# GameTechDev/Intel-Texture-Works-Plugin

Measured on AMD Instinct MI355X. Metric: Mpixels/s encode (BC1/BC3/BC7/BC6H) at 4k x 4k; bit-exact vs the oracle under the pinned ISPC sse/avx-target arithmetic model (no ispc binary exists here; sensitivity of that model: profiles/arith_sensitivity.txt), higher is better.
Workload: dtype f32; 1 GPU; bc7_slow: BC7 GetProfile_slow on ONE synthetic 4096x4096 RGBA8 surface, weak-sharded over 1 GPU(s) by block-row bands (4096 texel rows per rank), texels resident in HBM, device-pointer C ABI call; blocks_per_gpu=1048576, ranks_seen_by_rccl=1, device=gfx950:sramecc+:xnack- / AMD Radeon Graphics / 256 CUs / 2400 MHz, lib=itw-amd 0.1 gfx950 arith=x86-lut-nr contract=off

## Files before the change

intel-texture-works-plugin_amd/csrc/bc7.hip:

```cpp
#include <atomic>
#include <cstdlib>
#include <cstring>
#include <type_traits>
#include "bc7_exact.hpp"
#include "kernels.hpp"
#include "host_rt.hpp"
#ifdef ITW_TEST_HOOKS
#include "../../include/itw_test_hooks.h"
#endif

namespace itw {

#define BCN_TABLE_QUAL __device__ const
#include "bc7_f02_schedule.h"
#undef BCN_TABLE_QUAL

constexpr int LANE_PAL_LEVELS = 24;
constexpr int TPB = 256;
constexpr float INV255 = 1.0f / 255.0f;
constexpr int32_t ERR_MAX = 0x7fffffff;
enum Family { F_MODES02 = 0, F_MODES13 = 1, F_MODE7 = 2, F_MODES456 = 3 };

struct ModeTraits { int pairs, bits, ch; };
__device__ __forceinline__ constexpr ModeTraits traits(int mode)
// ... 1190 lines not shown
    const int32_t chunk = sel_chunk(sel, chunk_i);
    const int32_t nact = (!FAM7 && rgb_list) ? *rgb_count : nblocks;
    if (chunk * TPB >= nact) return;
    Lane ln;
    ln.T = stage_seed_tables_fast(s_seed16, s_seed32, threadIdx.x, TPB);
    __syncthreads();
    const int32_t gid = chunk * TPB + threadIdx.x;
    const bool live = gid < nact;
    const int32_t slot = live ? gid : nact - 1;
    const int32_t b = (!FAM7 && rgb_list) ? rgb_list[slot] : slot;
    ln.keys = nullptr;
    ln.pal = s_pal + threadIdx.x;
    load_block<VEC16>(ln.tx, src, stride, blocks_x, b);
    const int kind = tasks.kind[t];
    Win wa, wb;
    if (!FAM7 && kind == WK_SCAN02) {
        search_02(ln, S, wa, wb);
        if (live) { wins4[(int64_t)wide_win_slot(0) * nblocks + b] = pack_win(wa); if (!S.skip_mode2) wins4[(int64_t)wide_win_slot(2) * nblocks + b] = pack_win(wb); }
    } else if (!FAM7) {
        if (RANKED_LISTS && ranked13) search_two_subset<false, 3, 2>(ln, S, wa, wb); else search_two_subset<false, 3, 0>(ln, S, wa, wb);
        if (live) { wins4[(int64_t)wide_win_slot(1) * nblocks + b] = pack_win(wa); wins4[(int64_t)wide_win_slot(3) * nblocks + b] = pack_win(wb); }
    } else {
        if (S.channels == 4) { if (RANKED_LISTS && ranked7) search_two_subset<true, 4, 2>(ln, S, wa, wb); else search_two_subset<true, 4, 0>(ln, S, wa, wb); }
        else                 { if (RANKED_LISTS && ranked7) search_two_subset<true, 3, 2>(ln, S, wa, wb); else search_two_subset<true, 3, 0>(ln, S, wa, wb); }
        if (live) wins4[(int64_t)wide_win_slot(7) * nblocks + b] = pack_win(wa);
    }
}

__device__ __forceinline__ int32_t append_to_list(int32_t* __restrict__ list, int32_t* __restrict__ count, bool need, int32_t b)
{
    const unsigned long long m = __ballot(need);
    int32_t pos = -1;
    if (m) {
        const int lane = (int)(threadIdx.x & 63u);
        int32_t base = 0;
        if (lane == 0) base = atomicAdd(count, (int32_t)__popcll(m));
        base = __shfl(base, 0);
        if (need) { pos = base + (int32_t)__popcll(m & ((1ull << lane) - 1ull)); list[pos] = b; }
    }
    return pos;
}
__device__ __forceinline__ void append_to_rotation_lists(int32_t (*s_cnt)[4], const RotRegion& R, bool need0, bool need1, bool need2, int32_t b)
{
    const int lane = (int)__builtin_amdgcn_mbcnt_hi(~0u, __builtin_amdgcn_mbcnt_lo(~0u, 0u));
    const int wave = __builtin_amdgcn_readfirstlane((int)(threadIdx.x >> 6));
    const unsigned long long m0 = __ballot(need0), m1 = __ballot(need1), m2 = __ballot(need2);
    if (lane < 3) s_cnt[wave][lane] = (int32_t)__popcll(lane == 0 ? m0 : (lane == 1 ? m1 : m2));
    __syncthreads();
    if (threadIdx.x < 3u) {
        int32_t t = 0;
#pragma unroll
        for (int w = 0; w < TPB / 64; w++) t += s_cnt[w][lane];
        int32_t base = t ? atomicAdd(R.counts + lane, t) : 0;
#pragma unroll
        for (int w = 0; w < TPB / 64; w++) { const int32_t c = s_cnt[w][lane]; s_cnt[w][lane] = base; base += c; }
    }
    __syncthreads();
    const unsigned long long below = (1ull << lane) - 1ull;
    if (need0) R.lists[                      s_cnt[wave][0] + (int32_t)__popcll(m0 & below)] = b;
    if (need1) R.lists[(int64_t)R.cap     + s_cnt[wave][1] + (int32_t)__popcll(m1 & below)] = b;
    if (need2) R.lists[(int64_t)R.cap * 2 + s_cnt[wave][2] + (int32_t)__popcll(m2 & below)] = b;
}

__device__ __forceinline__ bool mode6_cannot_win(Lane& ln)
{
    if (__all(ln.best_err == 0)) return true;
    IStats<3> full;
    stats_int<3>(full, ln.tx.pl, whole_block());
    const float d = __builtin_amdgcn_sqrtf(subset_residual_bound(full) * rcp_of_count(16)) * 0.999999f - BOUND_SLACK3[16];
    const float e = fmaxf(d, 0.0f);
    const float lb = e * e * 0.999999f;
    return __all(lb >= (float)ln.best_err);
}

#ifndef FINISH_ALL_WAVES
#define FINISH_ALL_WAVES 2
#endif
#ifndef BOUND_BAIL_AFTER
#define BOUND_BAIL_AFTER 4
#endif
#ifndef BOUND_BAIL_LANES
#define BOUND_BAIL_LANES 40
#endif
template <bool VEC16, int PHASE>
__global__ void __launch_bounds__(TPB) __attribute__((amdgpu_waves_per_eu(FINISH_ALL_WAVES, FINISH_ALL_WAVES)))
bc7_finish_all(const uint8_t* __restrict__ src, int64_t stride, int32_t blocks_x, int32_t nblocks, uint8_t* __restrict__ dst,
               const uint32_t* __restrict__ wins4, const bc7_enc_settings S, int32_t* __restrict__ inc_err,
               const int32_t* __restrict__ in_list, const int32_t* __restrict__ in_count, int32_t* __restrict__ out_list, int32_t* __restrict__ out_count,
               int32_t* __restrict__ out_list7, int32_t* __restrict__ out_count7, const ChunkSel sel,
               const uint4* __restrict__ in_compact, uint4* __restrict__ out_compact, const RotRegion R)
{
    constexpr bool LISTED = PHASE == 2 || PHASE == 4 || PHASE == 5 || PHASE == 7 || PHASE == 8;
    constexpr bool DO02 = PHASE == 0 || PHASE == 2 || PHASE == 3 || PHASE == 5 || PHASE == 9;
    constexpr bool TAIL3 = PHASE == 3 || PHASE == 10;
    constexpr bool DO13 = PHASE == 0 || PHASE == 2 || PHASE == 4;
    constexpr bool DO7 = PHASE == 0 || PHASE == 1;
    constexpr bool DO456 = PHASE == 0 || PHASE == 1 || PHASE == 3 || PHASE == 6;
    __shared__ unsigned short s_seed16[2048];
    __shared__ uint32_t s_seed32[2048];
    __shared__ uint2 s_pal[LANE_PAL_LEVELS * TPB];
    __shared__ int32_t s_at[TAIL3 ? TPB / 64 : 1][64];
    __shared__ int32_t s_listed[TPB / 64];
    __shared__ int32_t s_rot[PHASE == 9 ? TPB / 64 : 1][4];
    if (sel.gate && *sel.gate != sel.want) return;
    const int32_t nact = LISTED ? *in_count : nblocks;
    const int32_t chunk = LISTED ? (int32_t)blockIdx.x : sel_chunk(sel, (int32_t)blockIdx.x);
    if (chunk * TPB >= nact) return;
    Lane ln;
    ln.T = stage_seed_tables_fast(s_seed16, s_seed32, threadIdx.x, TPB);
    __syncthreads();
    const int32_t gid = chunk * TPB + threadIdx.x;
    const bool live = gid < nact;
    const int32_t slot = live ? gid : nact - 1;
    const int32_t b = LISTED ? in_list[slot] : slot;
    ln.keys = nullptr;
    ln.pal = s_pal + threadIdx.x;
    if (LISTED && in_compact) load_block_compact(ln.tx, in_compact, slot); else load_block<VEC16>(ln.tx, src, stride, blocks_x, b);
    ln.best_err = ERR_MAX;
    ln.best[0] = ln.best[1] = ln.best[2] = ln.best[3] = 0u;
    ln.improved = false;
    ln.opaque_err = 0;
    if (S.channels == 4) {
        uint32_t e = 0;
#pragma unroll
        for (int d = 0; d < 4; d++) { const uint32_t x = ~ln.tx.pl[3][d]; e = udot4(x, x, e); }
        ln.opaque_err = (int32_t)e;
    }
    const bool on13 = S.mode_selection[1];
    int32_t e_alpha = ERR_MAX;
    if (PHASE == 2 || PHASE == 5) e_alpha = inc_err[b];
    if (PHASE == 4 || PHASE == 7 || PHASE == 8 || PHASE == 10) ln.best_err = inc_err[b];
    Win w;
    if (DO02 && S.mode_selection[0]) {
        unpack_win(w, wins4[(int64_t)wide_win_slot(0) * nblocks + b]);
        refine_and_commit<0>(ln, w, S.refineIterations[0], S.channels);
        if (!S.skip_mode2) { ln.tx.fence(); unpack_win(w, wins4[(int64_t)wide_win_slot(2) * nblocks + b]); refine_and_commit<2>(ln, w, S.refineIterations[2], S.channels); }
    }
    const int32_t e02 = ln.best_err;
    if (PHASE == 9) {
        if (live) { inc_err[b] = e02; R.words[b] = ~0ull; }
        ln.tx.fence();
        IStats<3> full;
        stats_int<3>(full, ln.tx.pl, whole_block());
        const float lim = (float)e02 - 0.5f;
        const bool on45 = live && S.mode_selection[2];
        bool need[3];
#pragma unroll
        for (int r = 0; r < 3; r++) need[r] = on45 && r >= S.mode45_channel0 && !(rotation_bound(r, full) >= lim);
        append_to_rotation_lists(s_rot, R, need[0], need[1], need[2], b);
    }
    if (PHASE == 10) {
        const unsigned long long v = R.words[b];
        const int32_t e = (int32_t)(v >> 32);
        if (v != ~0ull && e < ln.best_err) {
            const uint4 p = R.payload[(int64_t)((v >> ROT_WORD_ROT_SHIFT) & 3ull) * R.cap + (int64_t)(v & ROT_WORD_POS_MASK)];
            ln.best_err = e; ln.improved = true;
            ln.best[0] = p.x; ln.best[1] = p.y; ln.best[2] = p.z; ln.best[3] = p.w;
        }
        ln.tx.fence();
        if (S.mode_selection[3] && !mode6_cannot_win(ln)) mode_6<3>(ln, S);
    }
    if (DO13 && PHASE != 4) {
        if (on13 && S.fastSkipTreshold_mode1 > 0) { ln.tx.fence(); unpack_win(w, wins4[(int64_t)wide_win_slot(1) * nblocks + b]); refine_and_commit<1>(ln, w, S.refineIterations[1], S.channels); }
        if (on13 && S.fastSkipTreshold_mode3 > 0) { ln.tx.fence(); unpack_win(w, wins4[(int64_t)wide_win_slot(3) * nblocks + b]); refine_and_commit<3>(ln, w, S.refineIterations[3], S.channels); }
    }
    if (PHASE == 4) {
        const int parts = list_scan_parts(nact, nblocks);
        if (S.fastSkipTreshold_mode1 > 0) { ln.tx.fence(); merge_packed_parts<3, 3>(w, ln, wins4 + (int64_t)wide_win_slot(1) * nblocks, nact, parts, slot); refine_and_commit<1>(ln, w, S.refineIterations[1], S.channels); }
        if (S.fastSkipTreshold_mode3 > 0) { ln.tx.fence(); merge_packed_parts<3, 3>(w, ln, wins4 + (int64_t)wide_win_slot(3) * nblocks, nact, parts, slot); refine_and_commit<3>(ln, w, S.refineIterations[3], S.channels); }
    }
    bool redo = false;
    if (PHASE == 8) {
        const unsigned long long* pw = reinterpret_cast<const unsigned long long*>(wins4) + 2 * (int64_t)slot;
        const int32_t inc = ln.best_err;
        const bool heavy = pw[0] == PAIR_WORD_HEAVY;
        redo = !heavy && *out_count7 != 0;
        const bool use = !heavy && !redo;
        const unsigned long long v1 = (use && S.fastSkipTreshold_mode1 > 0) ? pw[0] : ~0ull, v3 = (use && S.fastSkipTreshold_mode3 > 0) ? pw[1] : ~0ull;
        if (v1 != ~0ull) {
            ln.tx.fence();
            w.err = (int32_t)(v1 >> 32); w.key = (int32_t)(uint32_t)v1; w.shape = w.key & 63;
            const bool open = w.err + ln.opaque_err >= inc;
            const int32_t before = ln.best_err;
            refine_and_commit<1>(ln, w, S.refineIterations[1], S.channels);
            redo = redo || (open && ln.best_err < before);
        }
        if (v3 != ~0ull) {
            ln.tx.fence();
            w.err = (int32_t)(v3 >> 32); w.key = (int32_t)(uint32_t)v3; w.shape = w.key & 63;
            const bool open = w.err + ln.opaque_err >= inc;
            const int32_t before = ln.best_err;
            refine_and_commit<3>(ln, w, S.refineIterations[3], S.channels);
            redo = redo || (open && ln.best_err < before);
        }
        append_to_list(out_list, out_count, live && redo, b);
    }
    if (PHASE == 7) {
        const int parts = list_scan_parts(nact, nblocks);
        ln.tx.fence();
        merge_packed_parts<4, 4>(w, ln, wins4 + (int64_t)wide_win_slot(7) * nblocks, nact, parts, slot);
        refine_and_commit<7>(ln, w, S.refineIterations[7], S.channels);
    }
    if (DO7 && on13 && S.fastSkipTreshold_mode7 > 0) { ln.tx.fence(); unpack_win(w, wins4[(int64_t)wide_win_slot(7) * nblocks + b]); refine_and_commit<7>(ln, w, S.refineIterations[7], S.channels); }
    if (DO456) {
        ln.tx.fence();
        if (S.mode_selection[2]) modes_45(ln, S);
        if (S.mode_selection[3]) {
            if (S.channels == 4) mode_6<4>(ln, S);
            else if (!mode6_cannot_win(ln)) mode_6<3>(ln, S);
        }
    }
    if (PHASE == 1) {
        if (live) inc_err[b] = ln.best_err;
        append_to_list(out_list, out_count, live && ln.opaque_err <= ln.best_err, b);
    }
    if (PHASE == 6) {
        const bool rgb = ln.opaque_err <= ln.best_err;
        if (live) inc_err[b] = rgb ? ln.best_err : ln.best_err + 1;
        append_to_list(out_list, out_count, live && rgb, b);
        append_to_list(out_list7, out_count7, live && !rgb, b);
    }
    if (TAIL3 || PHASE == 5) {
        int32_t inc;
        if (TAIL3) inc = ln.best_err + (ln.best_err < e02 ? 1 : 0);
        else            inc = (e02 <= e_alpha) ? e02 : e_alpha + 1;
        if (live) inc_err[b] = inc;
        ln.tx.fence();
        IStats<3> full;
        stats_int<3>(full, ln.tx.pl, whole_block());
        const float lim = (float)(inc - ln.opaque_err) - 0.5f;
        const float lim7 = (float)inc - 0.5f;
        const bool with7 = PHASE == 5 && out_list7 != nullptr;
        const PairTarget* target = nullptr;
        if (TAIL3) target = reinterpret_cast<const PairTarget*>(out_count + (PAIR_CTR_TARGET - PAIR_CTR_LIST));
        const bool pairs = TAIL3 && target->P.words != nullptr;
        bool need = !live, need7 = !live || !with7;
        unsigned long long mine = 0, any = 0;
#pragma unroll 1
        for (int shape = 0; shape < 64; shape++) {
            if (!pairs) {
                if (__all(need && need7)) break;
                if (shape == BOUND_BAIL_AFTER && __popcll(__ballot(need && need7)) >= BOUND_BAIL_LANES) { need = true; need7 = true; break; }
            }
            const float lb = two_subset_bound(shape, ln.tx.pl, full);
            const bool in = !(lb >= lim);
            need = need || in;
            need7 = need7 || !(lb >= lim7);
            if (pairs) {
                mine |= (live && in) ? (1ull << shape) : 0ull;
                any |= __ballot(live && in) ? (1ull << shape) : 0ull;
            }
        }
        int32_t pos = -1;
        if (!pairs) pos = append_to_list(out_list, out_count, live && need, b);
        else {
            const int lane = (int)__builtin_amdgcn_mbcnt_hi(~0u, __builtin_amdgcn_mbcnt_lo(~0u, 0u));
            const int wave = __builtin_amdgcn_readfirstlane((int)(threadIdx.x >> 6));
            const PairRegion P = target->P;
            const bool heavy = __popcll(mine) > PAIR_MAX_PER_BLOCK;
            if (heavy) mine = 0;
            const unsigned long long listed = __ballot(live && need);
            int32_t k = 0;
            for (unsigned long long rest = any; rest; rest &= rest - 1ull) {
                const int shape = __builtin_amdgcn_readfirstlane((int)__builtin_ctzll(rest));
                const int32_t c = (int32_t)__popcll(__ballot((mine >> shape) & 1ull));
                k = (lane == shape) ? c : k;
            }
            s_at[wave][lane] = k;
            if (lane == 0) s_listed[wave] = (int32_t)__popcll(listed);
            __syncthreads();
            if (threadIdx.x < 64u) {
                int32_t t = 0;
#pragma unroll
                for (int w = 0; w < TPB / 64; w++) t += s_at[w][lane];
                int32_t base = t ? atomicAdd(P.ctr + lane, t) : 0;
                if (base + t > P.cap) { P.ctr[PAIR_CTR_OVERFLOW] = 1; base = -1; }
#pragma unroll
                for (int w = 0; w < TPB / 64; w++) { const int32_t c = s_at[w][lane]; s_at[w][lane] = base; base = base < 0 ? -1 : base + c; }
            } else if (threadIdx.x == 64u) {
                int32_t t = 0;
#pragma unroll
                for (int w = 0; w < TPB / 64; w++) t += s_listed[w];
                int32_t base = t ? atomicAdd(out_count, t) : 0;
#pragma unroll
                for (int w = 0; w < TPB / 64; w++) { const int32_t c = s_listed[w]; s_listed[w] = base; base += c; }
            }
            __syncthreads();
            if (live && need) { pos = s_listed[wave] + (int32_t)__popcll(listed & ((1ull << lane) - 1ull)); out_list[pos] = b; }
            if (pos >= 0) { P.words[2 * (int64_t)pos] = heavy ? PAIR_WORD_HEAVY : ~0ull; P.words[2 * (int64_t)pos + 1] = ~0ull; }
            append_to_list(target->redo, P.ctr + PAIR_CTR_REDO, heavy, b);
            const int32_t at = s_at[wave][lane];
            for (unsigned long long rest = any; rest; rest &= rest - 1ull) {
                const int shape = __builtin_amdgcn_readfirstlane((int)__builtin_ctzll(rest));
                const bool in = (mine >> shape) & 1ull;
                const unsigned long long m = __ballot(in);
                const int32_t base = __builtin_amdgcn_readlane(at, shape);
                if (in && base >= 0) P.buckets[(int64_t)shape * P.cap + base + (int32_t)__popcll(m & ((1ull << lane) - 1ull))] = pos;
            }
        }
        if (out_compact && pos >= 0) {
            uint4* c = out_compact + (int64_t)pos * 4;
#pragma unroll
            for (int y = 0; y < 4; y++) c[y] = make_uint4(ln.tx.w[y * 4 + 0], ln.tx.w[y * 4 + 1], ln.tx.w[y * 4 + 2], ln.tx.w[y * 4 + 3]);
        }
        if (with7) append_to_list(out_list7, out_count7, live && need7, b);
    }
    bool store = live;
    if (PHASE == 2 || PHASE == 5) store = store && ln.best_err <= e_alpha;
    if (PHASE == 4 || PHASE == 7 || PHASE == 10) store = store && ln.improved;
    if (PHASE == 8) store = store && ln.improved && !redo;
    if ((PHASE == 4 || PHASE == 8) && store) inc_err[b] = ln.best_err;
    if (store) {
        uint32_t* d = reinterpret_cast<uint32_t*>(dst + (int64_t)b * 16);
        if (VEC16) *reinterpret_cast<uint4*>(d) = make_uint4(ln.best[0], ln.best[1], ln.best[2], ln.best[3]);
        else { d[0] = ln.best[0]; d[1] = ln.best[1]; d[2] = ln.best[2]; d[3] = ln.best[3]; }
    }
}

template <bool VEC16>
__global__ void __launch_bounds__(TPB)
bc7_pilot_estimate(const uint8_t* __restrict__ src, int64_t stride, int32_t blocks_x, int32_t nblocks, const uint32_t* __restrict__ wins4,
                   const int skip_mode2, const ChunkSel sel, int32_t* __restrict__ counters , const int32_t thr256,
                   int32_t* __restrict__ flag, int32_t* __restrict__ host_counts )
{
    const int32_t chunk = sel_chunk(sel, (int32_t)blockIdx.x * 8 + 3);
    if (chunk * TPB < nblocks) {
        const int32_t gid = chunk * TPB + threadIdx.x;
        const bool live = gid < nblocks;
        const int32_t b = live ? gid : nblocks - 1;
        Tex tx;
        load_block<VEC16>(tx, src, stride, blocks_x, b);
        Win w0, w2;
        unpack_win(w0, wins4[(int64_t)wide_win_slot(0) * nblocks + b]);
        unpack_win(w2, skip_mode2 ? 0xffffffffu : wins4[(int64_t)wide_win_slot(2) * nblocks + b]);
        const int32_t e = min(w0.err, w2.err);
        IStats<3> full;
        stats_int<3>(full, tx.pl, whole_block());
        const float lim = (float)e - 0.5f;
        bool need = !live;
#pragma unroll 1
        for (int shape = 0; shape < 64; shape++) {
            if (__all(need)) break;
            if (shape == BOUND_BAIL_AFTER && __popcll(__ballot(need)) >= BOUND_BAIL_LANES) { need = true; break; }
            need = need || !(two_subset_bound(shape, tx.pl, full) >= lim);
        }
        const unsigned long long ml = __ballot(live && need), mt = __ballot(live);
        if ((threadIdx.x & 63u) == 0u) { atomicAdd(counters + PILOT_LISTED, (int32_t)__popcll(ml)); atomicAdd(counters + PILOT_SAMPLED, (int32_t)__popcll(mt)); }
    }
    __syncthreads();
    if (threadIdx.x == 0) {
        __threadfence();
        if (atomicAdd(counters + PILOT_DONE, 1) == (int32_t)gridDim.x - 1) {
            __threadfence();
            const int64_t listed = atomicAdd(counters + PILOT_LISTED, 0), sampled = atomicAdd(counters + PILOT_SAMPLED, 0);
            *flag = (listed * 256 <= (int64_t)thr256 * sampled) ? 1 : 0;
            if (host_counts) { host_counts[0] = (int32_t)listed; host_counts[1] = (int32_t)sampled; __threadfence_system(); }
        }
    }
}

__global__ void __launch_bounds__(TPB) bc7_bounded_setup(int32_t* __restrict__ counters, const PairTarget t0, const PairTarget t1)
{
    for (int i = (int)threadIdx.x; i < CTR_WORDS + 2 * PAIR_CTR_WORDS; i += TPB) {
        const int j = i < CTR_WORDS ? 0 : (i - CTR_WORDS) % PAIR_CTR_WORDS;
        if (i < CTR_WORDS || j < PAIR_CTR_TARGET) counters[i] = 0;
    }
    if (threadIdx.x == 0) {
        *reinterpret_cast<PairTarget*>(counters + CTR_WORDS + PAIR_CTR_TARGET) = t0;
        *reinterpret_cast<PairTarget*>(counters + CTR_WORDS + PAIR_CTR_WORDS + PAIR_CTR_TARGET) = t1;
    }
}


__global__ void __launch_bounds__(TPB) __attribute__((amdgpu_waves_per_eu(4, 4)))
bc7_pair_scan(const uint8_t* __restrict__ src, int64_t stride, int32_t blocks_x, const int32_t* __restrict__ list, const uint4* __restrict__ compact,
              const bc7_enc_settings S, const PairRegion P)
{
    __shared__ unsigned short s_seed16[2048];
    __shared__ uint32_t s_seed32[2048];
    __shared__ uint2 s_pal[12 * TPB];
    __shared__ int32_t s_first[65];
    if (P.ctr[PAIR_CTR_OVERFLOW]) return;
    if (threadIdx.x == 0) {
        int32_t t = 0;
        for (int s = 0; s < 64; s++) { s_first[s] = t; t += (P.ctr[s] + 63) >> 6; }
        s_first[64] = t;
    }
    __syncthreads();
    const int32_t total = s_first[64];
    const int32_t wpb = TPB / 64;
    if ((int32_t)blockIdx.x * wpb >= total) return;
    Lane ln;
    ln.T = stage_seed_tables_fast(s_seed16, s_seed32, threadIdx.x, TPB);
    __syncthreads();
    ln.keys = nullptr;
    ln.pal = s_pal + threadIdx.x;
    const int lane = (int)(threadIdx.x & 63u);
    const bool on_a = S.fastSkipTreshold_mode1 > 0, on_b = S.fastSkipTreshold_mode3 > 0;
    int shape = 0;
// ... 573 lines not shown
    uint32_t* wins4;
    int32_t* alpha_err;
    int32_t* list_rgb;
    int32_t* list13;
    int32_t* list7;
    int32_t* ctr;
};
static Fused fused_context(const Bc7Launch& L, const Bc7Modes& M, float* workspace, const Bc7Aux* aux)
{
    Fused C{L, M, aux, fused_layout((size_t)L.n, fused_needs(M)), (int32_t)(((int64_t)L.n + TPB - 1) / TPB)};
    C.wins4 = reinterpret_cast<uint32_t*>(workspace);
    auto at = [&](size_t word) { return reinterpret_cast<int32_t*>(C.wins4 + word); };
    C.alpha_err = at(C.W.inc); C.list_rgb = at(C.W.list0); C.list13 = at(C.W.list1); C.list7 = at(C.W.list2); C.ctr = at(C.W.counts);
    return C;
}

struct Span { ChunkSel sel; int32_t cnt; hipStream_t s; uint32_t* wins; int32_t rows; };
struct BlockList { const int32_t* list; const int32_t* count; const uint4* compact; };
static const ChunkSel ALL_CHUNKS{0, 1, 0, nullptr, 0};
static const BlockList NO_LIST{nullptr, nullptr, nullptr};

struct Band {
    ChunkSel sel; int32_t cnt; hipStream_t s; int32_t* list; int32_t* count; uint32_t* wins; int32_t rows;
    int32_t* list_rgb; int32_t* count_rgb; int32_t* list7; int32_t* count7;
    uint4* compact; PairRegion P; int32_t* redo; RotRegion R;
};
static bool two_bands(const Fused& C) { return bc7_bands() > 1 && C.aux && !C.aux->single && C.aux->stream && C.nchunks >= 32; }
static Band make_band(const Fused& C, bool two, int k, hipStream_t s)
{
    int32_t stripe = C.nchunks / 16;
    stripe = stripe < 1 ? 1 : (stripe > 64 ? 64 : stripe);
    const int32_t stripes = (C.nchunks + stripe - 1) / stripe;
    Band B{};
    B.sel = ChunkSel{two ? 1 : 0, stripe, k, nullptr, 0};
    B.cnt = two ? ((stripes + 1 - k) / 2) * stripe : C.nchunks;
    B.s = s;
    B.wins = two ? C.wins4 + C.W.band[k].wins : C.wins4;
    B.rows = two ? B.cnt * TPB : C.L.n;
    return B;
}
static Span surface(const Fused& C) { return Span{ALL_CHUNKS, C.nchunks, C.L.st, C.wins4, C.L.n}; }
static Span band_chunks(const Fused& C, const Band& B) { return Span{B.sel, B.cnt, B.s, C.wins4, C.L.n}; }
static Span band_list(const Band& B) { return Span{ALL_CHUNKS, B.cnt, B.s, B.wins, B.rows}; }
static Span band_list_surface_rows(const Fused& C, const Band& B) { return Span{ALL_CHUNKS, B.cnt, B.s, C.wins4, C.L.n}; }

enum { SCAN02 = 1, SCAN13 = 2 };
static void scan_rgb(const Fused& C, int families, const Span& sp, const BlockList& in = NO_LIST, int32_t split = 0)
{
    const Bc7Launch& L = C.L;
    ScanTasks T{};
    if (C.M.on13 && (families & SCAN13)) T.kind[T.n++] = WK_SCAN13;
    if (C.M.on02 && (families & SCAN02)) T.kind[T.n++] = WK_SCAN02;
    if (T.n == 0) return;
    const int32_t c8 = ((sp.cnt + 7) / 8) * 8;
    const int32_t grain = c8 < 256 ? c8 : 256;
    const int32_t groups = (c8 + grain - 1) / grain;
    const dim3 grid((unsigned)(groups * grain * T.n));
    with_bools(L.vec, C.M.r13, [&](auto V, auto K) {
        hipLaunchKernelGGL((bc7_scan_all<decltype(V)::value, decltype(K)::value, false>), grid, dim3(TPB), 0, sp.s, L.src, L.stride, L.bx, sp.rows, sp.wins, L.S, T,
                           C.M.r13 ? 1 : 0, C.M.r7 ? 1 : 0, sp.cnt, grain, in.list, in.count, split, sp.sel, in.compact);
    });
}
static void scan_7(const Fused& C, const Span& sp, const BlockList& in = NO_LIST, int32_t split = 0)
{
    const Bc7Launch& L = C.L;
    if (!C.M.on7) return;
    const ScanTasks T7{1, {WK_SCAN7}};
    const int32_t chunks8 = ((sp.cnt + 7) / 8) * 8;
    with_bools(L.vec, C.M.r7, [&](auto V, auto K) {
        hipLaunchKernelGGL((bc7_scan_all<decltype(V)::value, decltype(K)::value, true>), dim3((unsigned)chunks8), dim3(TPB), 0, sp.s, L.src, L.stride, L.bx, sp.rows, sp.wins, L.S, T7,
                           C.M.r13 ? 1 : 0, C.M.r7 ? 1 : 0, sp.cnt, chunks8, in.list, in.count, split, ALL_CHUNKS, (const uint4*)nullptr);
    });
}
struct FinishIO {
    const int32_t* in_list = nullptr; const int32_t* in_count = nullptr; const uint4* in_compact = nullptr;
    int32_t* out_list = nullptr; int32_t* out_count = nullptr; uint4* out_compact = nullptr;
    int32_t* out_list7 = nullptr; int32_t* out_count7 = nullptr;
    RotRegion rot{nullptr, nullptr, nullptr, nullptr, 0};
    FinishIO& in(const int32_t* l, const int32_t* c, const uint4* texels = nullptr) { in_list = l; in_count = c; in_compact = texels; return *this; }
    FinishIO& out(int32_t* l, int32_t* c, uint4* texels = nullptr) { out_list = l; out_count = c; out_compact = texels; return *this; }
    FinishIO& out7(int32_t* l, int32_t* c) { out_list7 = l; out_count7 = c; return *this; }
    FinishIO& rotations(const RotRegion& r) { rot = r; return *this; }
};
template <int PH>
static void finish(const Fused& C, const Span& sp, const FinishIO& io = FinishIO())
{
    const Bc7Launch& L = C.L;
    const int32_t* band0 = C.ctr + CTR_WORDS + PAIR_CTR_LIST;
    if ((PH == 3 || PH == 10) && io.out_count != band0 && io.out_count != band0 + PAIR_CTR_WORDS)
        fail_msg("bc7_finish_all<3>: the list length must be word %d of a band's counter block", PAIR_CTR_LIST);
    with_bool(L.vec, [&](auto V) {
        hipLaunchKernelGGL((bc7_finish_all<decltype(V)::value, PH>), dim3((unsigned)sp.cnt), dim3(TPB), 0, sp.s, L.src, L.stride, L.bx, sp.rows, L.dst, sp.wins, L.S, C.alpha_err,
                           io.in_list, io.in_count, io.out_list, io.out_count, io.out_list7, io.out_count7, sp.sel, io.in_compact, io.out_compact, io.rot);
    });
}

static void launch_alpha_first_bounded7(const Fused& C)
{
    const Bc7Aux* aux = C.aux;
    hipStream_t st = C.L.st;
    ITW_CHECK(hipMemsetAsync(C.ctr, 0, CTR_WORDS * sizeof(int32_t), st));
    const bool two = two_bands(C);
    if (two) ITW_ROUTE_SEEN(ITW_ROUTE_TWO_BANDS);
    auto chain = [&](int k, hipStream_t s) {
        Band B = make_band(C, two, k, s);
        const size_t share = two ? k * C.W.band[0].cap : 0;
        int32_t* lengths = C.ctr + (k ? CTR_BAND1 : 0);
        B.list_rgb = C.list_rgb + share; B.count_rgb = lengths + CTR_LIST_RGB;
        B.list = C.list13 + share;       B.count = lengths + CTR_LIST_13;
        B.list7 = C.list7 + share;       B.count7 = lengths + CTR_LIST_7;
        const BlockList rgb{B.list_rgb, B.count_rgb, nullptr}, l13{B.list, B.count, nullptr}, l7{B.list7, B.count7, nullptr};
        finish<6>(C, band_chunks(C, B), FinishIO().out(B.list_rgb, B.count_rgb).out7(B.list7, B.count7));
        scan_rgb(C, SCAN02, band_list_surface_rows(C, B), rgb);
        finish<5>(C, band_list_surface_rows(C, B), FinishIO().in(B.list_rgb, B.count_rgb).out(B.list, B.count).out7(B.list7, B.count7));
        scan_rgb(C, SCAN13, band_list(B), l13, 1);
        finish<4>(C, band_list(B), FinishIO().in(B.list, B.count));
        scan_7(C, band_list(B), l7, 1);
        finish<7>(C, band_list(B), FinishIO().in(B.list7, B.count7));
    };
    if (!two) { chain(0, st); return; }
    ITW_CHECK(hipEventRecord(aux->fork, st));
    ITW_CHECK(hipStreamWaitEvent(aux->stream, aux->fork, 0));
    chain(1, aux->stream);
    chain(0, st);
    ITW_CHECK(hipEventRecord(aux->join, aux->stream));
    ITW_CHECK(hipStreamWaitEvent(st, aux->join, 0));
}

static void launch_alpha_first(const Fused& C)
{
    ITW_CHECK(hipMemsetAsync(C.ctr, 0, CTR_WORDS * sizeof(int32_t), C.L.st));
    const Span all = surface(C);
    int32_t* count_rgb = C.ctr + CTR_LIST_RGB; int32_t* count13 = C.ctr + CTR_LIST_13;
    const BlockList rgb{C.list_rgb, count_rgb, nullptr}, l13{C.list13, count13, nullptr};
    scan_7(C, all);
    finish<1>(C, all, FinishIO().out(C.list_rgb, count_rgb));
    if (C.M.bounded) {
        scan_rgb(C, SCAN02, all, rgb);
        finish<5>(C, all, FinishIO().in(C.list_rgb, count_rgb).out(C.list13, count13));
        scan_rgb(C, SCAN13, all, l13, 1);
        finish<4>(C, all, FinishIO().in(C.list13, count13));
    } else {
        scan_rgb(C, SCAN02 | SCAN13, all, rgb);
        finish<2>(C, all, FinishIO().in(C.list_rgb, count_rgb));
    }
}

struct RgbRoute { bool two, pairs, rot_tasks, pilot; };

static Band rgb_band(const Fused& C, const RgbRoute& R, int k, hipStream_t s)
{
    const ListRegion& r = C.W.band[k];
    uint32_t* w = C.wins4;
    Band B = make_band(C, R.two, k, s);
    B.list = R.two ? reinterpret_cast<int32_t*>(w + r.list) : C.list13;
    B.compact = env_once(ENV_COMPACT) ? reinterpret_cast<uint4*>(w + r.compact) : nullptr;
    B.P = PairRegion{reinterpret_cast<uint64_t*>(w + r.pair_words), reinterpret_cast<int32_t*>(w + r.pair_buckets), reinterpret_cast<int32_t*>(w + r.pair_ctr),
                     bc7_pair_cap((int32_t)(R.two ? r.pair_cap : 2 * r.pair_cap))};
    B.count = B.P.ctr + PAIR_CTR_LIST;
    B.redo = reinterpret_cast<int32_t*>(w + r.pair_redo);
    B.R = RotRegion{reinterpret_cast<int32_t*>(w + r.rot_lists), C.ctr + (k ? CTR_BAND1 : CTR_ROT), reinterpret_cast<unsigned long long*>(w + C.W.rot_words),
                    reinterpret_cast<uint4*>(w + r.rot_payload), (int32_t)(R.two ? r.cap : 2 * r.cap)};
    return B;
}
static void rgb_setup(const Fused& C, const RgbRoute& R, const Band& A, const Band& B)
{
    const PairTarget off{PairRegion{nullptr, nullptr, nullptr, 0}, nullptr};
    hipLaunchKernelGGL(bc7_bounded_setup, dim3(1), dim3(TPB), 0, C.L.st, C.ctr, R.pairs ? PairTarget{A.P, A.redo} : off, R.pairs ? PairTarget{B.P, B.redo} : off);
}
static void rgb_head(const Fused& C, const Band& B) { scan_rgb(C, SCAN02, band_chunks(C, B)); }
static void rgb_pilot(const Fused& C, const Band& B, int32_t thr256, int32_t* host_counts)
{
    const Bc7Launch& L = C.L;
    with_bool(L.vec, [&](auto V) {
        hipLaunchKernelGGL((bc7_pilot_estimate<decltype(V)::value>), dim3((unsigned)((B.cnt + 7) / 8)), dim3(TPB), 0, L.st, L.src, L.stride, L.bx, L.n, C.wins4,
                           L.S.skip_mode2 ? 1 : 0, B.sel, C.ctr + CTR_PILOT, thr256, C.ctr + CTR_PILOT_FLAG, host_counts);
    });
}
static void rgb_tail(const Fused& C, const RgbRoute& R, const Band& B)
{
    const Bc7Launch& L = C.L;
    auto gated = [&](int32_t want) { Span g = band_chunks(C, B); if (R.pilot) { g.sel.gate = C.ctr + CTR_PILOT_FLAG; g.sel.want = want; } return g; };
    if (R.rot_tasks) {
        finish<9>(C, gated(1), FinishIO().rotations(B.R));
        with_bool(L.vec, [&](auto V) { hipLaunchKernelGGL((bc7_rot_tasks<decltype(V)::value>), dim3((unsigned)B.cnt), dim3(TPB), 0, B.s, L.src, L.stride, L.bx, L.S, C.alpha_err, B.R); });
        finish<10>(C, gated(1), FinishIO().out(B.list, B.count, B.compact).rotations(B.R));
    } else
        finish<3>(C, gated(1), FinishIO().out(B.list, B.count, B.compact));
    if (R.pairs) {
        int32_t* redo_count = B.P.ctr + PAIR_CTR_REDO;
        const Span pair_words{ALL_CHUNKS, B.cnt, B.s, reinterpret_cast<uint32_t*>(B.P.words), B.rows};
        hipLaunchKernelGGL(bc7_pair_scan, dim3((unsigned)((B.cnt + 1) / 2)), dim3(TPB), 0, B.s, L.src, L.stride, L.bx, B.list, B.compact, L.S, B.P);
        finish<8>(C, pair_words, FinishIO().in(B.list, B.count, B.compact).out(B.redo, redo_count).out7(nullptr, B.P.ctr + PAIR_CTR_OVERFLOW));
        scan_rgb(C, SCAN13, band_list(B), BlockList{B.redo, redo_count, nullptr}, 1);
        finish<4>(C, band_list(B), FinishIO().in(B.redo, redo_count));
    } else {
        scan_rgb(C, SCAN13, band_list(B), BlockList{B.list, B.count, B.compact}, 1);
        finish<4>(C, band_list(B), FinishIO().in(B.list, B.count, B.compact));
    }
    if (R.pilot) {
        scan_rgb(C, SCAN13, gated(0));
        finish<0>(C, gated(0));
    }
}
static void rgb_print_counters(const Fused& C, const RgbRoute& R, const Band& A, const Band& B)
{
    int32_t h[CTR_WORDS + 2 * PAIR_CTR_WORDS];
    ITW_CHECK(hipStreamSynchronize(C.L.st));
    ITW_CHECK(hipMemcpy(h, C.ctr, sizeof h, hipMemcpyDeviceToHost));
    const int32_t* p = h + CTR_PILOT; const int32_t* r0 = h + CTR_ROT; const int32_t* r1 = h + CTR_BAND1;
    std::fprintf(stderr, "bc7 pilot: estimate %d of %d sampled blocks listed -> %s; lists %d + %d of %lld blocks\n", p[PILOT_LISTED], p[PILOT_SAMPLED],
                 h[CTR_PILOT_FLAG] ? "bounded" : "reference order", h[CTR_WORDS + PAIR_CTR_LIST], h[CTR_WORDS + PAIR_CTR_WORDS + PAIR_CTR_LIST], (long long)C.L.n);
    if (R.rot_tasks) std::fprintf(stderr, "bc7 rot tasks: rotation lists %d / %d / %d (band 0) + %d / %d / %d (band 1)\n", r0[0], r0[1], r0[2], r1[0], r1[1], r1[2]);
    for (int k = 0; k < 2 && R.pairs; k++) {
        const PairRegion& P = (k ? B : A).P;
        int32_t c[PAIR_CTR_WORDS];
        ITW_CHECK(hipMemcpy(c, P.ctr, sizeof c, hipMemcpyDeviceToHost));
        long long sum = 0; int32_t top = 0;
        for (int i = 0; i < 64; i++) { sum += c[i]; top = c[i] > top ? c[i] : top; }
        std::fprintf(stderr, "bc7 pairs: band %d: %lld pairs, fullest bucket %d of %d, overflow %d, deferred to the full scan %d\n", k, sum, top, P.cap,
                     c[PAIR_CTR_OVERFLOW], c[PAIR_CTR_REDO]);
    }
}
static void launch_rgb_bounded(const Fused& C)
{
    const Bc7Aux* aux = C.aux;
    hipStream_t st = C.L.st;
    const bool two = two_bands(C), rotations_ok = C.M.channels == 3 && C.L.S.mode45_channel0 >= 0 && C.L.S.mode45_channel0 <= 3;
    const bool pairs = env_every_call(ENV_PAIRS), rot_tasks = env_every_call(ENV_ROT_TASKS) && rotations_ok;
    const RgbRoute R{two, pairs, rot_tasks, two && bc7_pilot_threshold() >= 0 && aux->mid};
    if (R.two) ITW_ROUTE_SEEN(ITW_ROUTE_TWO_BANDS);
    if (R.pilot) ITW_ROUTE_SEEN(ITW_ROUTE_PILOT);
    if (R.pairs) ITW_ROUTE_SEEN(ITW_ROUTE_PAIRS);
    if (R.rot_tasks) ITW_ROUTE_SEEN(ITW_ROUTE_ROT_TASKS);
    if (!R.two) {
        const Band B = rgb_band(C, R, 0, st);
        if (B.compact) ITW_ROUTE_SEEN(ITW_ROUTE_COMPACT);
        rgb_setup(C, R, B, B);
        const bool verdict = aux && aux->verdict && aux->verdict->event;
        const bool probe = verdict && aux->probe;
        if (verdict) ITW_ROUTE_SEEN(ITW_ROUTE_HOST_VERDICT);
        if (probe) ITW_ROUTE_SEEN(ITW_ROUTE_PROBE);
        if (probe) scan_rgb(C, SCAN02, Span{ChunkSel{2, 1, 0, nullptr, 0}, (C.nchunks + 7) / 8, st, C.wins4, C.L.n});
        else rgb_head(C, B);
        if (verdict) {
            rgb_pilot(C, B, 256, aux->verdict->host_counts_dev);
            ITW_CHECK(hipEventRecord(aux->verdict->event, st));
            aux->verdict->valid = true;
        }
        if (!probe) rgb_tail(C, R, B);
        return;
    }
    hipStream_t s2 = aux->stream;
    const Band A = rgb_band(C, R, 0, st), B = rgb_band(C, R, 1, s2);
    if (A.compact && B.compact) ITW_ROUTE_SEEN(ITW_ROUTE_COMPACT);
    rgb_setup(C, R, A, B);
    ITW_CHECK(hipEventRecord(aux->fork, st));
    ITW_CHECK(hipStreamWaitEvent(s2, aux->fork, 0));
    rgb_head(C, B); rgb_head(C, A);
    if (R.pilot) {
        rgb_pilot(C, A, bc7_pilot_threshold(), nullptr);
        ITW_CHECK(hipEventRecord(aux->mid, st));
        ITW_CHECK(hipStreamWaitEvent(s2, aux->mid, 0));
    }
    rgb_tail(C, R, B); rgb_tail(C, R, A);
    ITW_CHECK(hipEventRecord(aux->join, s2));
    ITW_CHECK(hipStreamWaitEvent(st, aux->join, 0));
    if (env_once(ENV_PILOT_DEBUG)) rgb_print_counters(C, R, A, B);
#ifdef ITW_TEST_HOOKS
    if (g_counters_armed.load(std::memory_order_relaxed)) {
        int32_t h[CTR_WORDS + 2 * PAIR_CTR_WORDS], out[ITW_BC7_CALL_COUNTERS] = {};
        ITW_CHECK(hipStreamSynchronize(st));
        ITW_CHECK(hipMemcpy(h, C.ctr, sizeof h, hipMemcpyDeviceToHost));
        out[ITW_BC7_CC_PILOT_LISTED] = h[CTR_PILOT + PILOT_LISTED]; out[ITW_BC7_CC_PILOT_SAMPLED] = h[CTR_PILOT + PILOT_SAMPLED]; out[ITW_BC7_CC_PILOT_FLAG] = h[CTR_PILOT_FLAG];
        for (int k = 0; k < 2; k++) {
            const int32_t* band = h + CTR_WORDS + k * PAIR_CTR_WORDS;
            for (int r = 0; r < 3; r++) out[ITW_BC7_CC_ROT_LISTS + 3 * k + r] = h[(k ? CTR_BAND1 : CTR_ROT) + r];
            out[ITW_BC7_CC_LISTED + k] = band[PAIR_CTR_LIST];
            for (int s = 0; s < 64; s++) out[ITW_BC7_CC_PAIRS + k] += band[s];
            out[ITW_BC7_CC_OVERFLOW + k] = band[PAIR_CTR_OVERFLOW];
            out[ITW_BC7_CC_REDO + k] = band[PAIR_CTR_REDO];
        }
        for (int i = 0; i < ITW_BC7_CALL_COUNTERS; i++) g_call_counters[i].store(out[i], std::memory_order_relaxed);
    }
#endif
}

static void launch_reference_order(const Fused& C)
{
    scan_rgb(C, SCAN02 | SCAN13, surface(C));
    scan_7(C, surface(C));
    finish<0>(C, surface(C));
}

template <int FAMILY>
static void launch_ranked_family(Bc7Launch& L, bool ranked, bool long_list)
{
    if (!ranked) launch_search<FAMILY, 0>(L);
    else if (long_list) launch_search<FAMILY, 1>(L);
    else launch_search<FAMILY, 2>(L);
    launch_finish<FAMILY>(L);
}
static void launch_per_family(Bc7Launch& L, const Bc7Modes& M)
{
    if (M.on02) { launch_search<F_MODES02, 0>(L); launch_finish<F_MODES02>(L); }
    if (M.on13) launch_ranked_family<F_MODES13>(L, M.r13, M.long13);
    if (M.on7) launch_ranked_family<F_MODE7>(L, M.r7, M.long7);
    if (M.on45 || M.on6) launch_finish<F_MODES456>(L);
    if (L.first) ITW_CHECK(hipMemsetAsync(L.dst, 0, (size_t)L.n * 16, L.st));
}

void launch_bc7(const uint8_t* src, int64_t stride, int width, int height, uint8_t* dst,
                const bc7_enc_settings& s, float* workspace, hipStream_t st, const Bc7Aux* aux)
{
    const int bx = width / 4, by = height / 4;
    const int64_t n = (int64_t)bx * by;
    if (n <= 0) return;
    const Bc7Modes M = bc7_modes(s);
    Bc7Launch L;
    L.S = s;
    L.S.channels = M.channels;
    L.err = reinterpret_cast<int32_t*>(workspace);
    L.wins = reinterpret_cast<uint4*>(reinterpret_cast<uint8_t*>(workspace) + (((size_t)n * sizeof(int32_t) + 15) & ~(size_t)15));
    L.vec = ((reinterpret_cast<uintptr_t>(src) | (uintptr_t)stride | reinterpret_cast<uintptr_t>(dst)) & 15) == 0;
    L.grid = dim3((unsigned)((n + TPB - 1) / TPB));
    L.st = st; L.src = src; L.stride = stride; L.bx = bx; L.n = (int32_t)n; L.dst = dst; L.first = 1;
    const bool single = aux && aux->single;
    if (aux && aux->probe && !has_order_verdict(M)) { ITW_ROUTE_SEEN(ITW_ROUTE_PROBE_IGNORED); return; }
    if (!single && bc7_use_wide(n, L.S, M, aux ? aux->wide_max_blocks : 0)) { ITW_ROUTE_SEEN(ITW_ROUTE_WIDE); launch_bc7_wide(L, M, workspace, aux); return; }
    if (!env_once(ENV_FUSED) || M.long13 || M.long7 || !M.any()) { ITW_ROUTE_SEEN(ITW_ROUTE_PER_FAMILY); launch_per_family(L, M); return; }
    const Fused C = fused_context(L, M, workspace, aux);
    if (M.alpha_first && M.bounded && M.on7 && !M.r7 && (M.on45 || M.on6)) { ITW_ROUTE_SEEN(ITW_ROUTE_ALPHA_FIRST_BOUNDED7); launch_alpha_first_bounded7(C); }
    else if (M.alpha_first) { ITW_ROUTE_SEEN(M.bounded ? ITW_ROUTE_ALPHA_FIRST_BOUNDED : ITW_ROUTE_ALPHA_FIRST_PLAIN); launch_alpha_first(C); }
    else if (M.rgb_bounded) { ITW_ROUTE_SEEN(ITW_ROUTE_RGB_BOUNDED); launch_rgb_bounded(C); }
    else { ITW_ROUTE_SEEN(ITW_ROUTE_REFERENCE_ORDER); launch_reference_order(C); }
}

}
```

Baseline: 4262 Mpixels/s.

## Split rotation-path finish into finish kernel plus separate bound-list kernel

```diff
diff --git a/intel-texture-works-plugin_amd/csrc/bc7.hip b/intel-texture-works-plugin_amd/csrc/bc7.hip
--- a/intel-texture-works-plugin_amd/csrc/bc7.hip
+++ b/intel-texture-works-plugin_amd/csrc/bc7.hip
@@ -1296,8 +1296,101 @@
 #ifndef BOUND_BAIL_LANES
 #define BOUND_BAIL_LANES 40
 #endif
+template <bool TAIL3, int AT_ROWS>
+__device__ __forceinline__ void bounded_list_tail(Tex& tx, const int32_t inc, const int32_t opaque_err, const bool live, const int32_t b,
+                                                  int32_t (&s_at)[AT_ROWS][64], int32_t (&s_listed)[TPB / 64], int32_t* __restrict__ out_list, int32_t* __restrict__ out_count,
+                                                  int32_t* __restrict__ out_list7, int32_t* __restrict__ out_count7, uint4* __restrict__ out_compact)
+{
+    tx.fence();
+    IStats<3> full;
+    stats_int<3>(full, tx.pl, whole_block());
+    const float lim = (float)(inc - opaque_err) - 0.5f;
+    const float lim7 = (float)inc - 0.5f;
+    const bool with7 = !TAIL3 && out_list7 != nullptr;
+    const PairTarget* target = nullptr;
+    if (TAIL3) target = reinterpret_cast<const PairTarget*>(out_count + (PAIR_CTR_TARGET - PAIR_CTR_LIST));
+    const bool pairs = TAIL3 && target->P.words != nullptr;
+    bool need = !live, need7 = !live || !with7;
+    unsigned long long mine = 0, any = 0;
+#pragma unroll 1
+    for (int shape = 0; shape < 64; shape++) {
+        if (!pairs) {
+            if (__all(need && need7)) break;
+            if (shape == BOUND_BAIL_AFTER && __popcll(__ballot(need && need7)) >= BOUND_BAIL_LANES) { need = true; need7 = true; break; }
+        }
+        const float lb = two_subset_bound(shape, tx.pl, full);
+        const bool in = !(lb >= lim);
+        need = need || in;
+        need7 = need7 || !(lb >= lim7);
+        if (pairs) {
+            mine |= (live && in) ? (1ull << shape) : 0ull;
+            any |= __ballot(live && in) ? (1ull << shape) : 0ull;
+        }
+    }
+    int32_t pos = -1;
+    if (!pairs) pos = append_to_list(out_list, out_count, live && need, b);
+    else {
+        const int lane = (int)__builtin_amdgcn_mbcnt_hi(~0u, __builtin_amdgcn_mbcnt_lo(~0u, 0u));
+        const int wave = __builtin_amdgcn_readfirstlane((int)(threadIdx.x >> 6));
+        const PairRegion P = target->P;
+        const bool heavy = __popcll(mine) > PAIR_MAX_PER_BLOCK;
+        if (heavy) mine = 0;
+        const unsigned long long listed = __ballot(live && need);
+        int32_t k = 0;
+        for (unsigned long long rest = any; rest; rest &= rest - 1ull) {
+            const int shape = __builtin_amdgcn_readfirstlane((int)__builtin_ctzll(rest));
+            const int32_t c = (int32_t)__popcll(__ballot((mine >> shape) & 1ull));
+            k = (lane == shape) ? c : k;
+        }
+        s_at[wave][lane] = k;
+        if (lane == 0) s_listed[wave] = (int32_t)__popcll(listed);
+        __syncthreads();
+        if (threadIdx.x < 64u) {
+            int32_t t = 0;
+#pragma unroll
+            for (int w = 0; w < TPB / 64; w++) t += s_at[w][lane];
+            int32_t base = t ? atomicAdd(P.ctr + lane, t) : 0;
+            if (base + t > P.cap) { P.ctr[PAIR_CTR_OVERFLOW] = 1; base = -1; }
+#pragma unroll
+            for (int w = 0; w < TPB / 64; w++) { const int32_t c = s_at[w][lane]; s_at[w][lane] = base; base = base < 0 ? -1 : base + c; }
+        } else if (threadIdx.x == 64u) {
+            int32_t t = 0;
+#pragma unroll
+            for (int w = 0; w < TPB / 64; w++) t += s_listed[w];
+            int32_t base = t ? atomicAdd(out_count, t) : 0;
+#pragma unroll
+            for (int w = 0; w < TPB / 64; w++) { const int32_t c = s_listed[w]; s_listed[w] = base; base += c; }
+        }
+        __syncthreads();
+        if (live && need) { pos = s_listed[wave] + (int32_t)__popcll(listed & ((1ull << lane) - 1ull)); out_list[pos] = b; }
+        if (pos >= 0) { P.words[2 * (int64_t)pos] = heavy ? PAIR_WORD_HEAVY : ~0ull; P.words[2 * (int64_t)pos + 1] = ~0ull; }
+        append_to_list(target->redo, P.ctr + PAIR_CTR_REDO, heavy, b);
+        const int32_t at = s_at[wave][lane];
+        for (unsigned long long rest = any; rest; rest &= rest - 1ull) {
+            const int shape = __builtin_amdgcn_readfirstlane((int)__builtin_ctzll(rest));
+            const bool in = (mine >> shape) & 1ull;
+            const unsigned long long m = __ballot(in);
+            const int32_t base = __builtin_amdgcn_readlane(at, shape);
+            if (in && base >= 0) P.buckets[(int64_t)shape * P.cap + base + (int32_t)__popcll(m & ((1ull << lane) - 1ull))] = pos;
+        }
+    }
+    if (out_compact && pos >= 0) {
+        uint4* c = out_compact + (int64_t)pos * 4;
+#pragma unroll
+        for (int y = 0; y < 4; y++) c[y] = make_uint4(tx.w[y * 4 + 0], tx.w[y * 4 + 1], tx.w[y * 4 + 2], tx.w[y * 4 + 3]);
+    }
+    if (with7) append_to_list(out_list7, out_count7, live && need7, b);
+}
+
+#ifndef FINISH10_WAVES
+#define FINISH10_WAVES 3
+#endif
+#ifndef FINISH10_PAL_LEVELS
+#define FINISH10_PAL_LEVELS 16
+#endif
+__host__ __device__ constexpr int finish_all_waves(int phase) { return phase == 10 ? FINISH10_WAVES : FINISH_ALL_WAVES; }
 template <bool VEC16, int PHASE>
-__global__ void __launch_bounds__(TPB) __attribute__((amdgpu_waves_per_eu(FINISH_ALL_WAVES, FINISH_ALL_WAVES)))
+__global__ void __launch_bounds__(TPB) __attribute__((amdgpu_waves_per_eu(finish_all_waves(PHASE), finish_all_waves(PHASE))))
 bc7_finish_all(const uint8_t* __restrict__ src, int64_t stride, int32_t blocks_x, int32_t nblocks, uint8_t* __restrict__ dst,
                const uint32_t* __restrict__ wins4, const bc7_enc_settings S, int32_t* __restrict__ inc_err,
                const int32_t* __restrict__ in_list, const int32_t* __restrict__ in_count, int32_t* __restrict__ out_list, int32_t* __restrict__ out_count,
@@ -1312,8 +1405,8 @@
     constexpr bool DO456 = PHASE == 0 || PHASE == 1 || PHASE == 3 || PHASE == 6;
     __shared__ unsigned short s_seed16[2048];
     __shared__ uint32_t s_seed32[2048];
-    __shared__ uint2 s_pal[LANE_PAL_LEVELS * TPB];
-    __shared__ int32_t s_at[TAIL3 ? TPB / 64 : 1][64];
+    __shared__ uint2 s_pal[(PHASE == 10 ? FINISH10_PAL_LEVELS : LANE_PAL_LEVELS) * TPB];
+    __shared__ int32_t s_at[PHASE == 3 ? TPB / 64 : 1][64];
     __shared__ int32_t s_listed[TPB / 64];
     __shared__ int32_t s_rot[PHASE == 9 ? TPB / 64 : 1][4];
     if (sel.gate && *sel.gate != sel.want) return;
@@ -1439,85 +1532,7 @@
         if (TAIL3) inc = ln.best_err + (ln.best_err < e02 ? 1 : 0);
         else            inc = (e02 <= e_alpha) ? e02 : e_alpha + 1;
         if (live) inc_err[b] = inc;
-        ln.tx.fence();
-        IStats<3> full;
-        stats_int<3>(full, ln.tx.pl, whole_block());
-        const float lim = (float)(inc - ln.opaque_err) - 0.5f;
-        const float lim7 = (float)inc - 0.5f;
-        const bool with7 = PHASE == 5 && out_list7 != nullptr;
-        const PairTarget* target = nullptr;
-        if (TAIL3) target = reinterpret_cast<const PairTarget*>(out_count + (PAIR_CTR_TARGET - PAIR_CTR_LIST));
-        const bool pairs = TAIL3 && target->P.words != nullptr;
-        bool need = !live, need7 = !live || !with7;
-        unsigned long long mine = 0, any = 0;
-#pragma unroll 1
-        for (int shape = 0; shape < 64; shape++) {
-            if (!pairs) {
-                if (__all(need && need7)) break;
-                if (shape == BOUND_BAIL_AFTER && __popcll(__ballot(need && need7)) >= BOUND_BAIL_LANES) { need = true; need7 = true; break; }
-            }
-            const float lb = two_subset_bound(shape, ln.tx.pl, full);
-            const bool in = !(lb >= lim);
-            need = need || in;
-            need7 = need7 || !(lb >= lim7);
-            if (pairs) {
-                mine |= (live && in) ? (1ull << shape) : 0ull;
-                any |= __ballot(live && in) ? (1ull << shape) : 0ull;
-            }
-        }
-        int32_t pos = -1;
-        if (!pairs) pos = append_to_list(out_list, out_count, live && need, b);
-        else {
-            const int lane = (int)__builtin_amdgcn_mbcnt_hi(~0u, __builtin_amdgcn_mbcnt_lo(~0u, 0u));
-            const int wave = __builtin_amdgcn_readfirstlane((int)(threadIdx.x >> 6));
-            const PairRegion P = target->P;
-            const bool heavy = __popcll(mine) > PAIR_MAX_PER_BLOCK;
-            if (heavy) mine = 0;
-            const unsigned long long listed = __ballot(live && need);
-            int32_t k = 0;
-            for (unsigned long long rest = any; rest; rest &= rest - 1ull) {
-                const int shape = __builtin_amdgcn_readfirstlane((int)__builtin_ctzll(rest));
-                const int32_t c = (int32_t)__popcll(__ballot((mine >> shape) & 1ull));
-                k = (lane == shape) ? c : k;
-            }
-            s_at[wave][lane] = k;
-            if (lane == 0) s_listed[wave] = (int32_t)__popcll(listed);
-            __syncthreads();
-            if (threadIdx.x < 64u) {
-                int32_t t = 0;
-#pragma unroll
-                for (int w = 0; w < TPB / 64; w++) t += s_at[w][lane];
-                int32_t base = t ? atomicAdd(P.ctr + lane, t) : 0;
-                if (base + t > P.cap) { P.ctr[PAIR_CTR_OVERFLOW] = 1; base = -1; }
-#pragma unroll
-                for (int w = 0; w < TPB / 64; w++) { const int32_t c = s_at[w][lane]; s_at[w][lane] = base; base = base < 0 ? -1 : base + c; }
-            } else if (threadIdx.x == 64u) {
-                int32_t t = 0;
-#pragma unroll
-                for (int w = 0; w < TPB / 64; w++) t += s_listed[w];
-                int32_t base = t ? atomicAdd(out_count, t) : 0;
-#pragma unroll
-                for (int w = 0; w < TPB / 64; w++) { const int32_t c = s_listed[w]; s_listed[w] = base; base += c; }
-            }
-            __syncthreads();
-            if (live && need) { pos = s_listed[wave] + (int32_t)__popcll(listed & ((1ull << lane) - 1ull)); out_list[pos] = b; }
-            if (pos >= 0) { P.words[2 * (int64_t)pos] = heavy ? PAIR_WORD_HEAVY : ~0ull; P.words[2 * (int64_t)pos + 1] = ~0ull; }
-            append_to_list(target->redo, P.ctr + PAIR_CTR_REDO, heavy, b);
-            const int32_t at = s_at[wave][lane];
-            for (unsigned long long rest = any; rest; rest &= rest - 1ull) {
-                const int shape = __builtin_amdgcn_readfirstlane((int)__builtin_ctzll(rest));
-                const bool in = (mine >> shape) & 1ull;
-                const unsigned long long m = __ballot(in);
-                const int32_t base = __builtin_amdgcn_readlane(at, shape);
-                if (in && base >= 0) P.buckets[(int64_t)shape * P.cap + base + (int32_t)__popcll(m & ((1ull << lane) - 1ull))] = pos;
-            }
-        }
-        if (out_compact && pos >= 0) {
-            uint4* c = out_compact + (int64_t)pos * 4;
-#pragma unroll
-            for (int y = 0; y < 4; y++) c[y] = make_uint4(ln.tx.w[y * 4 + 0], ln.tx.w[y * 4 + 1], ln.tx.w[y * 4 + 2], ln.tx.w[y * 4 + 3]);
-        }
-        if (with7) append_to_list(out_list7, out_count7, live && need7, b);
+        if (PHASE != 10) bounded_list_tail<PHASE == 3>(ln.tx, inc, ln.opaque_err, live, b, s_at, s_listed, out_list, out_count, out_list7, out_count7, out_compact);
     }
     bool store = live;
     if (PHASE == 2 || PHASE == 5) store = store && ln.best_err <= e_alpha;
@@ -1529,6 +1544,34 @@
         if (VEC16) *reinterpret_cast<uint4*>(d) = make_uint4(ln.best[0], ln.best[1], ln.best[2], ln.best[3]);
         else { d[0] = ln.best[0]; d[1] = ln.best[1]; d[2] = ln.best[2]; d[3] = ln.best[3]; }
     }
+}
+
+#ifndef BOUND_LIST_WAVES
+#define BOUND_LIST_WAVES 6
+#endif
+template <bool VEC16>
+__global__ void __launch_bounds__(TPB) __attribute__((amdgpu_waves_per_eu(BOUND_LIST_WAVES, BOUND_LIST_WAVES)))
+bc7_bound_list(const uint8_t* __restrict__ src, int64_t stride, int32_t blocks_x, int32_t nblocks, const int32_t channels, const int32_t* __restrict__ inc_err,
+               int32_t* __restrict__ out_list, int32_t* __restrict__ out_count, const ChunkSel sel, uint4* __restrict__ out_compact)
+{
+    __shared__ int32_t s_at[TPB / 64][64];
+    __shared__ int32_t s_listed[TPB / 64];
+    if (sel.gate && *sel.gate != sel.want) return;
+    const int32_t chunk = sel_chunk(sel, (int32_t)blockIdx.x);
+    if (chunk * TPB >= nblocks) return;
+    const int32_t gid = chunk * TPB + threadIdx.x;
+    const bool live = gid < nblocks;
+    const int32_t b = live ? gid : nblocks - 1;
+    Tex tx;
+    load_block<VEC16>(tx, src, stride, blocks_x, b);
+    int32_t opaque_err = 0;
+    if (channels == 4) {
+        uint32_t e = 0;
+#pragma unroll
+        for (int d = 0; d < 4; d++) { const uint32_t x = ~tx.pl[3][d]; e = udot4(x, x, e); }
+        opaque_err = (int32_t)e;
+    }
+    bounded_list_tail<true>(tx, inc_err[b], opaque_err, live, b, s_at, s_listed, out_list, out_count, nullptr, nullptr, out_compact);
 }
 
 template <bool VEC16>
@@ -2268,16 +2311,28 @@
     FinishIO& out7(int32_t* l, int32_t* c) { out_list7 = l; out_count7 = c; return *this; }
     FinishIO& rotations(const RotRegion& r) { rot = r; return *this; }
 };
+static bool band_list_length(const Fused& C, const int32_t* count)
+{
+    const int32_t* band0 = C.ctr + CTR_WORDS + PAIR_CTR_LIST;
+    return count == band0 || count == band0 + PAIR_CTR_WORDS;
+}
 template <int PH>
 static void finish(const Fused& C, const Span& sp, const FinishIO& io = FinishIO())
 {
     const Bc7Launch& L = C.L;
-    const int32_t* band0 = C.ctr + CTR_WORDS + PAIR_CTR_LIST;
-    if ((PH == 3 || PH == 10) && io.out_count != band0 && io.out_count != band0 + PAIR_CTR_WORDS)
-        fail_msg("bc7_finish_all<3>: the list length must be word %d of a band's counter block", PAIR_CTR_LIST);
+    if (PH == 3 && !band_list_length(C, io.out_count)) fail_msg("bc7_finish_all<3>: the list length must be word %d of a band's counter block", PAIR_CTR_LIST);
     with_bool(L.vec, [&](auto V) {
         hipLaunchKernelGGL((bc7_finish_all<decltype(V)::value, PH>), dim3((unsigned)sp.cnt), dim3(TPB), 0, sp.s, L.src, L.stride, L.bx, sp.rows, L.dst, sp.wins, L.S, C.alpha_err,
                            io.in_list, io.in_count, io.out_list, io.out_count, io.out_list7, io.out_count7, sp.sel, io.in_compact, io.out_compact, io.rot);
+    });
+}
+static void bound_list(const Fused& C, const Span& sp, const FinishIO& io)
+{
+    const Bc7Launch& L = C.L;
+    if (!band_list_length(C, io.out_count)) fail_msg("bc7_bound_list: the list length must be word %d of a band's counter block", PAIR_CTR_LIST);
+    with_bool(L.vec, [&](auto V) {
+        hipLaunchKernelGGL((bc7_bound_list<decltype(V)::value>), dim3((unsigned)sp.cnt), dim3(TPB), 0, sp.s, L.src, L.stride, L.bx, sp.rows, (int32_t)L.S.channels,
+                           (const int32_t*)C.alpha_err, io.out_list, io.out_count, sp.sel, io.out_compact);
     });
 }
 
@@ -2370,7 +2425,8 @@
     if (R.rot_tasks) {
         finish<9>(C, gated(1), FinishIO().rotations(B.R));
         with_bool(L.vec, [&](auto V) { hipLaunchKernelGGL((bc7_rot_tasks<decltype(V)::value>), dim3((unsigned)B.cnt), dim3(TPB), 0, B.s, L.src, L.stride, L.bx, L.S, C.alpha_err, B.R); });
-        finish<10>(C, gated(1), FinishIO().out(B.list, B.count, B.compact).rotations(B.R));
+        finish<10>(C, gated(1), FinishIO().rotations(B.R));
+        bound_list(C, gated(1), FinishIO().out(B.list, B.count, B.compact));
     } else
         finish<3>(C, gated(1), FinishIO().out(B.list, B.count, B.compact));
     if (R.pairs) {
@@ -2407,6 +2463,28 @@
         std::fprintf(stderr, "bc7 pairs: band %d: %lld pairs, fullest bucket %d of %d, overflow %d, deferred to the full scan %d\n", k, sum, top, P.cap,
                      c[PAIR_CTR_OVERFLOW], c[PAIR_CTR_REDO]);
     }
+}
+static void rgb_snapshot_counters(const Fused& C)
+{
+#ifdef ITW_TEST_HOOKS
+    if (g_counters_armed.load(std::memory_order_relaxed)) {
+        int32_t h[CTR_WORDS + 2 * PAIR_CTR_WORDS], out[ITW_BC7_CALL_COUNTERS] = {};
+        ITW_CHECK(hipStreamSynchronize(C.L.st));
+        ITW_CHECK(hipMemcpy(h, C.ctr, sizeof h, hipMemcpyDeviceToHost));
+        out[ITW_BC7_CC_PILOT_LISTED] = h[CTR_PILOT + PILOT_LISTED]; out[ITW_BC7_CC_PILOT_SAMPLED] = h[CTR_PILOT + PILOT_SAMPLED]; out[ITW_BC7_CC_PILOT_FLAG] = h[CTR_PILOT_FLAG];
+        for (int k = 0; k < 2; k++) {
+            const int32_t* band = h + CTR_WORDS + k * PAIR_CTR_WORDS;
+            for (int r = 0; r < 3; r++) out[ITW_BC7_CC_ROT_LISTS + 3 * k + r] = h[(k ? CTR_BAND1 : CTR_ROT) + r];
+            out[ITW_BC7_CC_LISTED + k] = band[PAIR_CTR_LIST];
+            for (int s = 0; s < 64; s++) out[ITW_BC7_CC_PAIRS + k] += band[s];
+            out[ITW_BC7_CC_OVERFLOW + k] = band[PAIR_CTR_OVERFLOW];
+            out[ITW_BC7_CC_REDO + k] = band[PAIR_CTR_REDO];
+        }
+        for (int i = 0; i < ITW_BC7_CALL_COUNTERS; i++) g_call_counters[i].store(out[i], std::memory_order_relaxed);
+    }
+#else
+    (void)C;
+#endif
 }
 static void launch_rgb_bounded(const Fused& C)
 {
@@ -2435,6 +2513,7 @@
             aux->verdict->valid = true;
         }
         if (!probe) rgb_tail(C, R, B);
+        rgb_snapshot_counters(C);
         return;
     }
     hipStream_t s2 = aux->stream;
@@ -2453,23 +2532,7 @@
     ITW_CHECK(hipEventRecord(aux->join, s2));
     ITW_CHECK(hipStreamWaitEvent(st, aux->join, 0));
     if (env_once(ENV_PILOT_DEBUG)) rgb_print_counters(C, R, A, B);
-#ifdef ITW_TEST_HOOKS
-    if (g_counters_armed.load(std::memory_order_relaxed)) {
-        int32_t h[CTR_WORDS + 2 * PAIR_CTR_WORDS], out[ITW_BC7_CALL_COUNTERS] = {};
-        ITW_CHECK(hipStreamSynchronize(st));
-        ITW_CHECK(hipMemcpy(h, C.ctr, sizeof h, hipMemcpyDeviceToHost));
-        out[ITW_BC7_CC_PILOT_LISTED] = h[CTR_PILOT + PILOT_LISTED]; out[ITW_BC7_CC_PILOT_SAMPLED] = h[CTR_PILOT + PILOT_SAMPLED]; out[ITW_BC7_CC_PILOT_FLAG] = h[CTR_PILOT_FLAG];
-        for (int k = 0; k < 2; k++) {
-            const int32_t* band = h + CTR_WORDS + k * PAIR_CTR_WORDS;
-            for (int r = 0; r < 3; r++) out[ITW_BC7_CC_ROT_LISTS + 3 * k + r] = h[(k ? CTR_BAND1 : CTR_ROT) + r];
-            out[ITW_BC7_CC_LISTED + k] = band[PAIR_CTR_LIST];
-            for (int s = 0; s < 64; s++) out[ITW_BC7_CC_PAIRS + k] += band[s];
-            out[ITW_BC7_CC_OVERFLOW + k] = band[PAIR_CTR_OVERFLOW];
-            out[ITW_BC7_CC_REDO + k] = band[PAIR_CTR_REDO];
-        }
-        for (int i = 0; i < ITW_BC7_CALL_COUNTERS; i++) g_call_counters[i].store(out[i], std::memory_order_relaxed);
-    }
-#endif
+    rgb_snapshot_counters(C);
 }
 
 static void launch_reference_order(const Fused& C)
```

Result: faster. 4345 Mpixels/s (median of 6 runs) (+1.9%).
